# connortannahill/MM-ADMM

Hardware: AMD Instinct MI355X
Metric: ADMM iterations/sec on 1M-node 2D mesh; achieved HBM GB/s in SpMV (higher is better)
Workload: dtype f64

## Files before the change

### mm-admm_amd/csrc/host/engine.cpp

```cpp
#include <algorithm>
#include <chrono>
#include <cmath>
#include <cstring>
#include <limits>
#include <memory>
#include <mutex>
#include <string>
#include <vector>

#include "../../../include/mmx_sparse.h"
#include "../kernels/admm_kernels.h"
#include "../kernels/field_kernels.h"
#include "../kernels/quality_kernels.h"
#include "../kernels/regrid_kernels.h"
#include "../kernels/slide_kernels.h"
#include "../kernels/state_kernels.h"
#include "../kernels/transfer_kernels.h"
#include "comm.h"
#include "common.h"
#include "partition.h"
#include "slide.h"
#include "state.h"
#include "transfer.h"
#include "xup_records.h"
// ... 223 lines not shown
            std::stable_sort(ord.begin() + lo, ord.begin() + hi, [&](int a, int b) { return key[a] < key[b]; });
          }
        } else {
          std::stable_sort(ord.begin(), ord.end(), [&](int a, int b) { return key[a] < key[b]; });
        }
      };
      order(inner);
      order(bound);
      std::vector<int32_t> ord(inner);
      ord.insert(ord.end(), bound.begin(), bound.end());
      nodeOrder_.upload(ord.data(), std::max<size_t>(ord.size(), 1), st_);
      XupRecords recs;
      if (knobs_.xupRec) {
        const int ch = std::max(D == 2 ? MMX_XU_CH2D : 8, knobs_.xupCh);
        recs = build_xup_records(nl, ord.data(), plan_.incPtr.data(), plan_.incSrc.data(), invdiag.data(), ch);
        xrec_.upload(recs.rec.data(), recs.rec.size(), st_);
        xinv_.upload(recs.invdiag.data(), recs.invdiag.size(), st_);
        xslot_.upload(recs.slot.data(), recs.slot.size(), st_);
        xslotStride_ = (int)recs.stride;
        xslotCh_ = ch;
        const int chs = D == 2 ? MMX_XU_CH2D : knobs_.xupCh;
        xupTail_ = 0;
        for (int v = 0; v < nl; ++v) xupTail_ += std::max(0, plan_.incPtr[v + 1] - plan_.incPtr[v] - chs);
      }
      streamWait();
    }
    invdiag_.upload(invdiag.data(), invdiag.size(), st_);
    if (compMesh_) Vc_.upload(Vcl.data(), Vcl.size(), st_);
    uploadGridCoords();
    gvals_.upload(grid_.vals.data(), grid_.vals.size(), st_);
    if (D == 3) {
      gpad_.alloc(gvals_.n / 9 * 10);
      launch_pad_rows(gvals_.p, (long long)(gvals_.n / 9), gpad_.p, st_);
    }
    updateIso();
    Vp_.upload(Vl.data(), Vl.size(), st_);
    x_.upload(Vl.data(), Vl.size(), st_);
    xPrev_.upload(Vl.data(), Vl.size(), st_);
    xBar_.upload(Vl.data(), Vl.size(), st_);
    if (nranks_ > 1) {
      expOff_.upload(plan_.sendOff.data(), std::max<size_t>(plan_.sendOff.size(), 1), st_);
      export_.alloc((size_t)std::max<size_t>(plan_.sendOff.size(), 1) * D);
      remote_.alloc((size_t)std::max(plan_.recvRows, 1) * D);
    }
    z_.alloc((size_t)nF_ * K * (kZUInterleaved ? 2 : 1));
    gcache_.alloc((size_t)nF_ * K);
// ... 71 lines not shown
      m_.zx = zsrc;
    else
      launch_gather_z<D>(m_, zsrc, z_.p, st_);
    gcacheValid_ = false;
    if (!zFromX) m_.zx = nullptr;
    StepScalars sc{prm_.tau, prm_.dt * prm_.dt, w_, dtOverTau};
    int nbx = 0, nbp = 0;
    if (fusePred) {
      m_.predPrev = xPrev_.p;
      m_.predBar = xBar_.p;
    }
    PackZX pz;
    if (zFromX) {
      pz.F = F_.p;
      pz.zx = zsrc;
      if (fusePred) {
        pz.x = x_.p;
        pz.xPrev = xPrev_.p;
      }
    }
    xupdateHalo(sc, &nbx, false, false, pz);
    m_.predPrev = m_.predBar = nullptr;
    const bool early = tol >= 0;
    int done = 0;
    double primal = 0, dual = 0;
    const bool deferRed = !early && nIters <= kDeferMax;
    const size_t slice = maxBlocks_ * kNumPartials;
    if (deferRed && partA_.n < slice * nIters) partA_.alloc(slice * std::max(nIters, 10));
    int firstDeferred = 0;
    hipEvent_t prevEnd = nullptr;
    for (int i = 0; i < nIters; ++i) {
      hipEvent_t a0 = nullptr, a1 = nullptr, b1 = nullptr;
      if (timing) {
        a0 = prevEnd;
        if (!a0) {
          a0 = nextEvent();
          MMX_HIP(hipEventRecord(a0, st_));
        }
      }
      const bool firstProx = !hessComputed_;
      const bool swapB = prox_double_buffered(D, knobs_.prox2dWave) && hessComputed_;
      if (hessComputed_) {
        tiePar_ ^= 1;
        std::swap(m_.tieCount, m_.tieStale);
      }
      m_.gcSkip = (D == 2 && knobs_.gcSkip && !early && i == nIters - 1) ? 1 : 0;
      launch_prox<D>(m_, knobs_, !hessComputed_, gcacheValid_, early ? tol / 100 : 1e-3 / 100, x_.p, z_.p, uPtr(), B_.p,
                     swapB ? B2_.p : B_.p, partA_.p + (deferRed ? slice * i : 0), &nbp, st_);
      m_.zx = nullptr;
      if (swapB) std::swap(B_.p, B2_.p);
      gcacheValid_ = !m_.gcSkip;
      if (timing) {
        a1 = nextEvent();
        MMX_HIP(hipEventRecord(a1, st_));
      }
      hessComputed_ = true;
      stepTaken_ = true;
      const bool resid = early || i == nIters - 1;
      xupdateHalo(sc, &nbx, resid, true, PackZX{});
      if (timing) {
        b1 = nextEvent();
        MMX_HIP(hipEventRecord(b1, st_));
        timed_.push_back({a0, a1, b1});
      }
      prevEnd = b1;
      if (deferRed) {
        if (firstProx && i < nIters - 1) {
          prevEnd = nullptr;
          launch_reduce_partials(partA_.p + slice * i, nbp, res_ + (size_t)i * 2 * kNumPartials, st_, red_);
          firstDeferred = i + 1;
        } else if (i == nIters - 1) {
          const int i0 = firstProx ? i : firstDeferred;
          launch_reduce_steps(partA_.p + slice * i0, slice, nbp, partB_.p, nbx, nIters - i0,
                              res_ + (size_t)i0 * 2 * kNumPartials, st_, red_);
        }
      } else if (resid) {
        prevEnd = nullptr;
        launch_reduce_partials2(partA_.p, nbp, res_ + (size_t)i * 2 * kNumPartials, partB_.p, nbx,
                                res_ + (size_t)i * 2 * kNumPartials + kNumPartials, st_, red_);
      } else {
        prevEnd = nullptr;
        launch_reduce_partials(partA_.p, nbp, res_ + (size_t)i * 2 * kNumPartials, st_, red_);
      }
      done = i + 1;
      if (early) {
        std::vector<double> rv;
        fetchResults(res_ + (size_t)i * 2 * kNumPartials, 1, rv);
        const double* r = rv.data();
        primal = sqrt(r[kNumPartials + 2]);
        dual = sqrt(r[1]);
        if (r[4] > 0 || (primal < tol && dual < tol)) break;
      }
    }
    if (slideOn_ && !slS_.sliding.empty()) {
      launch_slide_project<D>(slX0_.p, slFaces_.p, slStarPtr_.p, slStarFace_.p, slMask_.p, slIds_.p,
                              (int)slS_.sliding.size(), x_.p, slAnchor_.p, slStepCnt_.p, st_);
      slStepValid_ = true;
    }
    MMX_HIP(hipMemcpyAsync(Vp_.p, x_.p, (size_t)nP_ * D * sizeof(double), hipMemcpyDeviceToDevice, st_));
    vpVersion_++;
    if (timing) {
      eStep1 = nextEvent();
      MMX_HIP(hipEventRecord(eStep1, st_));
    }
    fetchResults(res_, done, hostRes_);
    MMX_HIP(hipGetLastError());
    bool bad = false;
    long long bf = 0;
    int mx = 0;
    for (int i = 0; i < done; ++i) {
      const double* r = &hostRes_[(size_t)i * 2 * kNumPartials];
      bad |= r[4] > 0;
      bf += (long long)r[3];
      mx = std::max(mx, (int)r[5]);
    }
#ifdef MMX_HINT_PROBE
    {
      double hits = 0;
      for (int i = 0; i < done; ++i) hits += hostRes_[(size_t)i * 2 * kNumPartials + 2];
      fprintf(stderr, "[hint-probe] step %lld: %.0f hits of %.0f lookups in %d proxes\n", (long long)stepsTaken_, hits,
              3.0 * nF_ * done, done);
    }
// ... 215 lines not shown
    if (n) *n = nP_;
    if (ids) std::memcpy(ids, plan_.localNodes.data(), plan_.localNodes.size() * sizeof(int32_t));
  }

  void sizes(int* nP, int* nF, int* gridRows) override {
    if (nP) *nP = nP_;
    if (nF) *nF = nF_;
    if (gridRows) *gridRows = (int)(grid_.vals.size() / (D * D));
  }

  void setTiming(bool on) override {
    resolveTimed();
    timing_ = on;
  }

  void stats(mmadmm_stats* s) override {
    resolveTimed();
    *s = st_stats_;
    const double nF = nF_, nP = nP_;
    const double ts = knobs_.tslot ? 1.0 : 0.0;
    s->prox_bytes = nF * (4.0 * (D + 1) + 1 + 8.0 * (2 * K + K * K) * 2 + 8.0 * K * 2 + ts * 8.0 * K) +
                    nP * 8.0 * D;
    const double ch = D == 2 ? MMX_XU_CH2D : knobs_.xupCh;
    const double fixed = knobs_.xupRec ? nP * (4.0 * kXupRecInts + 8.0 + 4.0 * ch) + 4.0 * (double)xupTail_
                                 : 4.0 * (nP + 1) + 4.0 * (D + 1) * nF + 8.0 * nP;
    s->xupdate_bytes = fixed + (16.0 - 8.0 * ts) * K * nF + 8.0 * D * nP * 2;
    s->monitor_iso = iso_ ? 1 : 0;
    s->halo_send_bytes = 8.0 * D * (double)plan_.sendOff.size();
    s->halo_recv_bytes = nranks_ > 1 ? 8.0 * D * (double)plan_.recvRows : 0.0;
    s->interior_nodes = nInner_;
    s->overlap = knobs_.overlap;
  }

  std::string options() const override { return knobs_.text(); }

  void resetStats() override {
    resolveTimed();
    const mmadmm_stats z{};
    st_stats_ = z;
  }

  void resolveTimed() {
    if (stepEv_.empty() && timed_.empty() && exEv_.empty()) return;
    streamWait();
    float ms = 0;
    for (auto& p : stepEv_) {
      MMX_HIP(hipEventElapsedTime(&ms, p.first, p.second));
      st_stats_.t_step_ms += ms;
// ... 1382 lines not shown
    m.inc_off = incOff_.p;
    m.remote = nranks_ > 1 ? remote_.p : nullptr;
    m.tslot = knobs_.tslot ? tslot_.p : nullptr;
    m.gcache = gcache_.p;
    m.tieList = tieList_.p;
    m.tieCount = tieCount_.p + tiePar_;
    m.tieStale = tieCount_.p + (tiePar_ ^ 1);
    m.invFlag = tieCount_.p + 2;
    m.nodeOrder = nodeOrder_.p;
    m.xupLo = 0;
    m.xupHi = nP_;
    m.prox2dWave = knobs_.prox2dWave;
    m.xupSweep = knobs_.xupSweep;
    m.xupCh = knobs_.xupCh;
    m.xupEarly = knobs_.xupEarly;
    m.forceTie = knobs_.forceTie;
    m.monHint = knobs_.monHint;
    if (knobs_.xupRec) {
      m.xrec = xrec_.p;
      m.xinv = xinv_.p;
      m.xslot = xslot_.p;
      m.xslotStride = xslotStride_;
      m.xslotCh = xslotCh_;
    }
    m.invdiag = invdiag_.p;
    m.Vc = compMesh_ ? Vc_.p : nullptr;
    m.gx = gx_.p;
    m.gy = gy_.p;
    m.gz = (D == 3) ? gz_.p : gy_.p;
    m.gvals = gvals_.p;
    m.gpad = (D == 3) ? gpad_.p : nullptr;
    for (int a = 0; a < 3; ++a) m.gcell[a] = (D == 3) ? gcell_[a].p : nullptr;
    m.giso = iso_ ? giso_.p : nullptr;
    m.gnx = grid_.nx;
    m.gny = grid_.ny;
    m.gnz = grid_.nz;
    m.ghx = grid_.gx[1] - grid_.gx[0];
    m.ghy = grid_.gy[1] - grid_.gy[0];
    m.ghz = (D == 3) ? grid_.gz[1] - grid_.gz[0] : 1.0;
    m.grhx = 1.0 / m.ghx;
    m.grhy = 1.0 / m.ghy;
    m.grhz = 1.0 / m.ghz;
    const int ns[3] = {grid_.nx, grid_.ny, grid_.nz};
    double* A[3] = {&m.gax, &m.gay, &m.gaz};
    double* SP[3] = {&m.gspx, &m.gspy, &m.gspz};
    double* NS[3] = {&m.gnsx, &m.gnsy, &m.gnsz};
// ... 116 lines not shown
  DevBuf<unsigned char> rgScan_;
  size_t rgScanBytes_ = 0;
  double* rgHost_ = nullptr;
  hipStream_t st_ = nullptr;
  hipStream_t st2_ = nullptr;
  hipEvent_t evProx_ = nullptr, evEx_ = nullptr;
  int nInner_ = 0;
  std::vector<std::pair<hipEvent_t, hipEvent_t>> exEv_;
  DevBuf<int32_t> F_, incPtr_, incOff_;
  DevBuf<double> tslot_;
  DevBuf<uint8_t> sbits_, interior_;
  DevBuf<double> gcell_[3];
  DevBuf<double> giso_;
  DevBuf<int> isoFlag_;
  bool iso_ = false;
  std::vector<double> gcellH_[3];
  DevBuf<double> invdiag_, Vc_, gx_, gy_, gz_, gvals_, Vp_, x_, xPrev_, xBar_, z_, u_, gs_, B_, B2_, gcache_, gpad_;
  DevBuf<double> partA_, partB_, results_, export_, remote_, resAll_, redScratch_;
  RedWork red_;
  DevBuf<int32_t> expOff_, tieList_, nodeOrder_;
  DevBuf<int32_t> xrec_, xslot_;
  DevBuf<double> xinv_;
  int xslotStride_ = 0, xslotCh_ = 0;
  long long xupTail_ = 0;
  DevBuf<unsigned> tieCount_;
  int tiePar_ = 0;
  Comm* comm_ = nullptr;
  int rank_ = 0, nranks_ = 1;
  int resultsCap_ = 0;
  std::vector<double> hostRes_;
  DeviceMesh<D> m_{};
  bool hessComputed_ = false, stepTaken_ = false, gcacheValid_ = false;
  mmx_matrix jac_ = nullptr;
  mmx_param_iter jprm_{};
  bool beStepTaken_ = false, jacFactored_ = false;
  long long vpVersion_ = 0, jacVp_ = -1;
  double jacDt_ = 0.0;
  DevBuf<int32_t> jia_, jja_;
  DevBuf<double> jval_, jraw_, dv_, xn_, rhs_, dx_;
  DevBuf<unsigned> fdWork_;
  int maxColNodes_ = 65;
  int stepsTaken_ = 0;
  size_t maxBlocks_ = 1;
  static constexpr int kDeferMax = 64;
  bool timing_ = false;
  std::vector<hipEvent_t> evPool_;
// ... 450 lines not shown
```

### mm-admm_amd/csrc/host/knobs.h

```cpp
#pragma once
#include <climits>
#include <cstdio>
#include <cstdlib>
#include <cstring>
#include <stdexcept>
#include <string>

namespace mmx {

constexpr int kTslot2dMax = 2 * 2048 * 64;
constexpr int kXupEarlyDefault = 1;
constexpr int kRedSplitMin = 4096;
constexpr int kProxBlock = 64;
constexpr int kSweepGrid = 128;
constexpr int kFacWaveChunk = 0;
constexpr int kChainImportLat = 8;
constexpr int kFacImpRows = 384;
constexpr int kFacRMax = 4;

inline int env_int(const char* name, int dflt, int lo = INT_MIN, int hi = INT_MAX) {
  const char* e = std::getenv(name);
  if (!e) return dflt;
  const int v = std::atoi(e);
  return v < lo ? lo : v > hi ? hi : v;
// ... 50 lines not shown
    buf[n] = 0;
  }
  return (int)s.size() + 1;
}
}

#define MMX_ENGINE_KNOBS(X) \
   \
   \
  X(int, tslot, "MMX_TSLOT", nullptr, env_flag("MMX_TSLOT", D == 3 || nF <= kTslot2dMax)) \
   \
  X(int, spin, "MMX_SPIN", nullptr, env_flag("MMX_SPIN", true)) \
   \
  X(int, zx, "MMX_ZX", nullptr, env_flag("MMX_ZX", true)) \
   \
  X(int, overlap, "MMX_OVERLAP", nullptr, nranks > 1 && env_flag("MMX_OVERLAP", true)) \
   \
  X(int, fusePred, "MMX_FUSE_PRED", nullptr, env_flag("MMX_FUSE_PRED", true)) \
   \
  X(int, gcSkip, "MMX_GC_SKIP", nullptr, env_flag("MMX_GC_SKIP", true)) \
   \
  X(int, xupOrder, "MMX_XUP_ORDER", nullptr, env_int("MMX_XUP_ORDER", D == 3) == 1) \
   \
  X(int, xupRec, "MMX_XUP_REC", nullptr, env_flag("MMX_XUP_REC", true)) \
   \
  X(int, xupCh, "MMX_XUP_CH", nullptr, knobs_detail::snap_xup_ch(env_int("MMX_XUP_CH", 8))) \
   \
   \
   \
  X(int, xupSweep, "MMX_XUP_SWEEP", nullptr, env_int("MMX_XUP_SWEEP", D == 3 ? 1 : (k.xupRec ? 2 : 0), 0)) \
   \
  X(int, xupEarly, "MMX_XUP_EARLY", nullptr, env_flag("MMX_XUP_EARLY", kXupEarlyDefault != 0)) \
   \
  X(int, xupSweepResid, "MMX_XUP_SWEEP_RESID", nullptr, env_flag("MMX_XUP_SWEEP_RESID", true)) \
   \
   \
  X(int, xcdMap, "MMX_XCD_MAP", nullptr, env_int("MMX_XCD_MAP", 1)) \
   \
  X(int, prox2dWave, "MMX_PROX2D", "lds|wave", D == 2 && env_word("MMX_PROX2D", "lds|wave")) \
   \
  X(int, prox3dQuad, "MMX_PROX3D", "wave|quad", env_word("MMX_PROX3D", "wave|quad")) \
   \
  X(int, proxBlock, "MMX_PROX_BLOCK", nullptr, knobs_detail::one_of3(env_int("MMX_PROX_BLOCK", 0), 64, 128, 256, kProxBlock)) \
   \
  X(int, gradCache, "MMX_GRAD_CACHE", nullptr, env_int("MMX_GRAD_CACHE", 1)) \
   \
  X(int, forceTie, "MMX_FORCE_TIE", nullptr, env_int("MMX_FORCE_TIE", 0)) \
// ... 121 lines not shown
```

### mm-admm_amd/csrc/host/xup_records.h

```cpp
#pragma once
#include <algorithm>
#include <cstddef>
#include <cstdint>
#include <vector>

#include "../kernels/layout.h"

namespace mmx {

struct XupRecords {
  int ch = 0;
  size_t stride = 0;
  std::vector<int32_t> rec;
  std::vector<double> invdiag;
  std::vector<int32_t> slot;
};

inline XupRecords build_xup_records(int nP, const int32_t* order, const int32_t* incPtr, const int32_t* incOff,
                                    const double* invdiag, int ch) {
  XupRecords r;
  r.ch = ch;
  r.stride = (std::max<size_t>((size_t)std::max(nP, 0), 1) + kXupStridePad - 1) / kXupStridePad * kXupStridePad;
  r.rec.assign(r.stride * kXupRecInts, 0);
  r.invdiag.assign(r.stride, 0.0);
  r.slot.assign((size_t)ch * r.stride, 0);
  for (int p = 0; p < nP; ++p) {
    const int32_t v = order ? order[p] : p;
    const int32_t b = incPtr[v], e = incPtr[v + 1];
    r.rec[(size_t)p * kXupRecInts + 0] = v;
    r.rec[(size_t)p * kXupRecInts + 1] = b;
    r.rec[(size_t)p * kXupRecInts + 2] = e;
    r.invdiag[p] = invdiag[v];
    if (e > b)
      for (int j = 0; j < ch; ++j) r.slot[(size_t)j * r.stride + p] = incOff[std::min(b + j, e - 1)];
  }
  return r;
}

}
```

### mm-admm_amd/csrc/kernels/admm_kernels.h

```cpp
#pragma once
#include <hip/hip_runtime.h>
#include <stdint.h>

#include "../host/knobs.h"
#include "layout.h"

namespace mmx {

constexpr int kNumPartials = kLayoutPartials;

template <int D>
struct DeviceMesh {
  int nP, nF;
  const int* F;
  const uint8_t* sbits;
  const uint8_t* nodeInterior;
  const int* inc_ptr;
  const int* inc_off;
  const double* remote;
  double* tslot;
  const double* zx;
  double* predPrev;
  double* predBar;
  double* gcache;
// ... 9 lines not shown
  int xupLo, xupHi;
  const double* invdiag;
  const int* xrec;
  const double* xinv;
  const int* xslot;
  int xslotStride, xslotCh;
  int xupEarly;
  int gcSkip;
  const double* Vc;
  const double* gx;
  const double* gy;
  const double* gz;
  const double* gvals;
  const double* gpad;
  const double* gcell[3];
  const double* giso;
  int gnx, gny, gnz;
  double ghx, ghy, ghz, grhx, grhy, grhz;
  double gax, gay, gaz, gspx, gspy, gspz, gnsx, gnsy, gnsz, grnsx, grnsy, grnsz;
  double Ehat[9];
  double powd, w;
  int compMesh;
  int prox2dWave;
};

struct StepScalars {
  double tau, dtsq, w, dt_over_tau;
};

template <int D>
void launch_gather_z(const DeviceMesh<D>& m, const double* x, double* z, hipStream_t st);
template <int D>
void launch_grad_simplex(const DeviceMesh<D>& m, const double* x, double* gs, bool zeroFixed,
                         double* partials, int* nblocks, hipStream_t st);
template <int D>
void launch_predict(const DeviceMesh<D>& m, const EngineKnobs& k, int mode, const double* gs, double* x, double* xPrev,
                    double* xBar, double dt_over_tau, hipStream_t st);
template <int D>
void launch_xupdate(const DeviceMesh<D>& m, const EngineKnobs& k, const StepScalars& sc, const double* xBar,
                    const double* z, const double* u, double* x, double* partials, int* nblocks,
                    bool resid, hipStream_t st, bool useTslot = false);
void launch_pad_rows(const double* vals, long long rows, double* pad, hipStream_t st);
template <int D>
void launch_iso_compact(const double* vals, long long points, double* iso, int* notIso, hipStream_t st);
template <int D>
void launch_bkinv_identity(int nF, double* B, hipStream_t st);
// ... 51 lines not shown
```

### mm-admm_amd/csrc/kernels/admm_kernels_step.hip

```cpp
#include "admm_common.h"

namespace mmx {
template <int D>
__global__ void __launch_bounds__(kBlock) k_gather_z(DeviceMesh<D> m, const double* __restrict__ x,
                                                      double* __restrict__ z) {
  constexpr int K = D * (D + 1);
  const int s = blockIdx.x * kBlock + threadIdx.x;
  if (s >= m.nF) return;
  int f[D + 1];
  loadVerts<D>(m, s, f);
  double v[K];
  gatherX<D>(x, f, v);
#pragma unroll
  for (int i = 0; i < K; ++i) z[zu_base<D>(s) + zu_i<D>(i)] = v[i];
}

template <int D, int ISO = -1>
__global__ void __launch_bounds__(kBlock) k_grad_simplex(DeviceMesh<D> m, const double* __restrict__ x,
                                                          double* __restrict__ gs, int zeroFixedRows,
                                                          double* __restrict__ partials) {
  constexpr int K = D * (D + 1);
  const int s = blockIdx.x * kBlock + threadIdx.x;
  double pv[5] = {0, 0, 0, 0, 0};
  if (s < m.nF) {
// ... 30 lines not shown
    for (int t = b; t < e; ++t) {
      const int off = m.inc_off[t];
      const double* src = (off >= 0) ? gs + off : m.remote + (size_t)(-1 - off) * D;
#pragma unroll
      for (int c = 0; c < D; ++c) g[c] += src[c];
    }
#pragma unroll
    for (int c = 0; c < D; ++c) xb[c] = xv[c] - dt_over_tau * g[c];
  } else {
#pragma unroll
    for (int c = 0; c < D; ++c) xb[c] = 2 * xv[c] - xPrev[(size_t)v * D + c];
  }
#pragma unroll
  for (int c = 0; c < D; ++c) {
    xBar[(size_t)v * D + c] = xb[c];
    xPrev[(size_t)v * D + c] = xv[c];
  }
}

template <int CH>
struct XupHead {
  int v, b, e;
  double inv;
  int off[CH];
};
template <int D, int CH>
__device__ __forceinline__ void xup_head_rec(const DeviceMesh<D>& m, int idx, XupHead<CH>& h) {
  const int* r = m.xrec + (size_t)idx * kXupRecInts;
  h.v = r[0];
  h.b = r[1];
  h.e = r[2];
  h.inv = m.xinv[idx];
#pragma unroll
  for (int j = 0; j < CH; ++j) h.off[j] = m.xslot[(size_t)j * m.xslotStride + idx];
}
template <int D, int CH>
__device__ __forceinline__ void xup_head_csr(const DeviceMesh<D>& m, int idx, XupHead<CH>& h) {
  h.v = m.nodeOrder ? m.nodeOrder[idx] : idx;
  h.b = m.inc_ptr[h.v];
  h.e = m.inc_ptr[h.v + 1];
  h.inv = m.invdiag[h.v];
#pragma unroll
  for (int j = 0; j < CH; ++j) h.off[j] = (h.e > h.b) ? m.inc_off[min(h.b + j, h.e - 1)] : 0;
}
template <int D, bool RESID, bool TS, int CH = 8, bool ZX = false, bool PRED = false, bool REM = false>
__device__ __forceinline__ void xupdate_node(const DeviceMesh<D>& m, const StepScalars& sc,
                                             const double* __restrict__ xBar, const double* __restrict__ z,
                                             const double* __restrict__ u, double* __restrict__ x,
                                             const XupHead<CH>& h, double (&pv)[3]) {
  {
    const int v = h.v, b = h.b, e = h.e;
    double acc[D];
#pragma unroll
    for (int c = 0; c < D; ++c) acc[c] = 0.0;
    double xb[D], zn[D];
    if constexpr (PRED) {
      double xv[D];
#pragma unroll
      for (int c = 0; c < D; ++c) {
        xv[c] = x[(size_t)v * D + c];
        xb[c] = 2 * xv[c] - m.predPrev[(size_t)v * D + c];
      }
#pragma unroll
      for (int c = 0; c < D; ++c) {
        m.predBar[(size_t)v * D + c] = xb[c];
        m.predPrev[(size_t)v * D + c] = xv[c];
      }
    } else {
#pragma unroll
      for (int c = 0; c < D; ++c) xb[c] = xBar[(size_t)v * D + c];
    }
    constexpr bool zv0 = ZX && !TS;
    if constexpr (zv0) {
      if constexpr (PRED) {
#pragma unroll
        for (int c = 0; c < D; ++c) zn[c] = xb[c];
      } else {
#pragma unroll
        for (int c = 0; c < D; ++c) zn[c] = m.zx[(size_t)v * D + c];
      }
    }
    const double inv = h.inv;
    auto addChunk = [&](int t0, const int(&off)[CH]) {
      double zv[CH][D], uv[CH][D];
#pragma unroll
      for (int j = 0; j < CH; ++j) {
        const bool loc = off[j] >= 0;
        if constexpr (TS) {
          const double* pt = loc ? m.tslot + off[j] : m.remote + (size_t)(-1 - off[j]) * D;
#pragma unroll
          for (int c = 0; c < D; ++c) zv[j][c] = pt[c];
        } else {
          const double* pz = loc ? z + zu_off<D>(off[j]) : m.remote + (size_t)(-1 - off[j]) * D;
          const double* pu = loc ? u + zu_off<D>(off[j]) : pz;
#pragma unroll
          for (int c = 0; c < D; ++c) {
            if constexpr (zv0 && REM)
              zv[j][c] = loc ? zn[c] : pz[c];
            else if constexpr (zv0)
              zv[j][c] = zn[c];
            else
              zv[j][c] = pz[c];
            uv[j][c] = pu[c];
          }
        }
      }
#pragma unroll
      for (int j = 0; j < CH; ++j) {
        if (t0 + j < e) {
#pragma unroll
          for (int c = 0; c < D; ++c) {
            if constexpr (TS)
              acc[c] += zv[j][c];
            else
              acc[c] += (off[j] >= 0) ? sc.w * (sc.w * (zv[j][c] - uv[j][c])) : zv[j][c];
          }
        }
      }
    };
    if (b < e) addChunk(b, h.off);
    for (int t0 = b + CH; t0 < e; t0 += CH) {
      int off[CH];
#pragma unroll
      for (int j = 0; j < CH; ++j) off[j] = m.inc_off[min(t0 + j, e - 1)];
      addChunk(t0, off);
    }
    double xn[D];
#pragma unroll
    for (int c = 0; c < D; ++c) {
      xn[c] = ((sc.tau * xb[c]) + sc.dtsq * acc[c]) * inv;
      x[(size_t)v * D + c] = xn[c];
    }
    if constexpr (RESID) {
      double r2 = 0.0;
      auto residChunk = [&](int t0, const int(&off)[CH]) {
        double zv[CH][D];
#pragma unroll
        for (int j = 0; j < CH; ++j) {
          const double* pz = z + zu_off<D>(off[j] >= 0 ? off[j] : 0);
#pragma unroll
          for (int c = 0; c < D; ++c) zv[j][c] = pz[c];
        }
#pragma unroll
        for (int j = 0; j < CH; ++j) {
          if (t0 + j < e && off[j] >= 0) {
#pragma unroll
            for (int c = 0; c < D; ++c) {
              const double d = xn[c] - zv[j][c];
              r2 += d * d;
            }
          }
        }
      };
      if (b < e) residChunk(b, h.off);
      for (int t0 = b + CH; t0 < e; t0 += CH) {
        int off[CH];
#pragma unroll
        for (int j = 0; j < CH; ++j) off[j] = m.inc_off[min(t0 + j, e - 1)];
        residChunk(t0, off);
      }
      pv[2] = r2;
    }
  }
}
template <int D, int CH, bool REC>
__device__ __forceinline__ void xup_head(const DeviceMesh<D>& m, int idx, XupHead<CH>& h) {
  if constexpr (REC)
    xup_head_rec<D, CH>(m, idx, h);
  else
    xup_head_csr<D, CH>(m, idx, h);
}
template <int D, bool RESID, bool TS, bool ZX = false, bool PRED = false, bool REM = false, bool REC = false>
__global__ void __launch_bounds__(kBlock) k_xupdate(DeviceMesh<D> m, StepScalars sc,
                                                     const double* __restrict__ xBar,
                                                     const double* __restrict__ z,
                                                     const double* __restrict__ u, double* __restrict__ x,
                                                     double* __restrict__ partials, int xcd) {
  constexpr int CH = (D == 2 ? MMX_XU_CH2D : 8);
  const int lb = logical_block(xcd);
  const int idx = m.xupLo + lb * kBlock + threadIdx.x;
  double pv[3] = {0, 0, 0};
  if (idx < m.xupHi) {
    XupHead<CH> h;
    xup_head<D, CH, REC>(m, idx, h);
    xupdate_node<D, RESID, TS, CH, ZX, PRED, REM>(m, sc, xBar, z, u, x, h, pv);
  }
  if constexpr (RESID) block_partials<3>(pv, partials, lb);
}
template <int D, bool TS, int CH, bool RESID = false, bool REC = false, bool EARLY = false>
__global__ void __launch_bounds__(kBlock) k_xupdate_sweep(DeviceMesh<D> m, StepScalars sc,
                                                           const double* __restrict__ xBar,
                                                           const double* __restrict__ z, const double* __restrict__ u,
                                                           double* __restrict__ x, int n8, double* __restrict__ partials) {
  static_assert(REC || !EARLY, "the early request reads the records");
  const int c = (int)(blockIdx.x % 8), w = (int)(blockIdx.x / 8), per = (int)(gridDim.x / 8);
  const int lo = m.xupLo + c * n8, hi = min(lo + n8, m.xupHi);
  double pv[3], r2 = 0.0;
  int idx = lo + w * kBlock + (int)threadIdx.x;
  if constexpr (EARLY) {
    XupHead<CH> cur, nxt;
    if (idx < hi) xup_head<D, CH, true>(m, idx, cur);
    nxt = cur;
    for (; idx < hi; idx += per * kBlock) {
      if (idx + per * kBlock < hi) xup_head<D, CH, true>(m, idx + per * kBlock, nxt);
      __builtin_amdgcn_sched_barrier(0);
      xupdate_node<D, RESID, TS, CH>(m, sc, xBar, z, u, x, cur, pv);
      if constexpr (RESID) r2 += pv[2];
      cur = nxt;
    }
  } else {
    for (; idx < hi; idx += per * kBlock) {
      XupHead<CH> h;
      xup_head<D, CH, REC>(m, idx, h);
      xupdate_node<D, RESID, TS, CH>(m, sc, xBar, z, u, x, h, pv);
      if constexpr (RESID) r2 += pv[2];
    }
  }
  if constexpr (RESID) {
    double q[3] = {0.0, 0.0, r2};
    block_partials<3>(q, partials, (int)blockIdx.x);
  }
}

template <int D, int ISO = -1>
__global__ void __launch_bounds__(kBlock) k_energy(DeviceMesh<D> m, const double* __restrict__ x,
                                                    double* __restrict__ partials) {
  constexpr int K = D * (D + 1);
  const int s = blockIdx.x * kBlock + threadIdx.x;
  double pv[5] = {0, 0, 0, 0, 0};
  if (s < m.nF) {
    int f[D + 1];
    loadVerts<D>(m, s, f);
    double z[K], xi[K], Igt;
    gatherX<D>(x, f, z);
    loadXi<D>(m, f, xi);
    const double e = blockGrad<D, false, false>(gridOf<D, ISO>(m), constsOf<D>(m), z, xi, nullptr, nullptr, Igt);
    pv[0] = e;
// ... 165 lines not shown
                       zeroFixedRows ? 1 : 0, partials);
  });
}
template <int D>
void launch_predict(const DeviceMesh<D>& m, const EngineKnobs& k, int mode, const double* gs, double* x,
                    double* xPrev, double* xBar, double dt_over_tau, hipStream_t st) {
  if (m.nP == 0) return;
  hipLaunchKernelGGL(k_predict<D>, dim3(nblk_xcd(m.nP, k.xcdMap)), dim3(kBlock), 0, st, m, mode, gs, x, xPrev, xBar,
                     dt_over_tau, k.xcdMap);
}
template <int D>
void launch_xupdate(const DeviceMesh<D>& m, const EngineKnobs& k, const StepScalars& sc, const double* xBar,
                    const double* z, const double* u, double* x, double* partials, int* nblocks, bool resid,
                    hipStream_t st, bool useTslot) {
  const int nsub = m.xupHi - m.xupLo;
  *nblocks = nblk_xcd(nsub, k.xcdMap);
  if (nsub <= 0) {
    *nblocks = 0;
    return;
  }
  const bool ts = useTslot && m.tslot;
  const bool rem = m.remote != nullptr;
  const bool rec = m.xrec != nullptr;
  auto needCols = [&](int ch) {
    if (rec && m.xslotCh < ch) throw std::logic_error("launch_xupdate: the slot table has fewer columns than the chunk");
  };
  if (m.zx && !resid && !ts) {
    needCols(D == 2 ? MMX_XU_CH2D : 8);
    dispatch_bool(m.predBar != nullptr, [&](auto pred) {
      dispatch_bool(rem, [&](auto r) {
        dispatch_bool(rec, [&](auto rc) {
          hipLaunchKernelGGL(
              (k_xupdate<D, false, false, true, decltype(pred)::value, decltype(r)::value, decltype(rc)::value>),
              dim3(*nblocks), dim3(kBlock), 0, st, m, sc, xBar, z, u, x, partials, k.xcdMap);
        });
      });
    });
    return;
  }
  if (m.predBar || m.predPrev)
    throw std::logic_error("launch_xupdate: predBar set for an x-update that cannot fuse predictX");
  const bool sweepResid = resid && ts && k.xupSweepResid;
  if (m.xupSweep > 0 && (!resid || sweepResid)) {
    const int n8 = ((nsub + kBlock - 1) / kBlock + 7) / 8 * kBlock;
    const dim3 g(256 * m.xupSweep);
    auto sweep = [&](auto tsT, auto chT, auto residT, double* part) {
      constexpr bool TS = decltype(tsT)::value, RS = decltype(residT)::value;
      constexpr int CH = decltype(chT)::value;
      needCols(CH);
      if (rec && m.xupEarly)
        hipLaunchKernelGGL((k_xupdate_sweep<D, TS, CH, RS, true, true>), g, dim3(kBlock), 0, st, m, sc, xBar, z, u, x, n8,
                           part);
      else if (rec)
        hipLaunchKernelGGL((k_xupdate_sweep<D, TS, CH, RS, true, false>), g, dim3(kBlock), 0, st, m, sc, xBar, z, u, x, n8,
                           part);
      else
        hipLaunchKernelGGL((k_xupdate_sweep<D, TS, CH, RS>), g, dim3(kBlock), 0, st, m, sc, xBar, z, u, x, n8, part);
    };
    using T = std::true_type;
    using F = std::false_type;
    if (sweepResid) {
      *nblocks = (int)g.x;
      sweep(T{}, std::integral_constant<int, 8>{}, T{}, partials);
    } else if (ts && m.xupCh >= 24)
      sweep(T{}, std::integral_constant<int, 24>{}, F{}, nullptr);
    else if (ts && m.xupCh >= 16)
      sweep(T{}, std::integral_constant<int, 16>{}, F{}, nullptr);
    else if (ts)
      sweep(T{}, std::integral_constant<int, 8>{}, F{}, nullptr);
    else
      sweep(F{}, std::integral_constant<int, (D == 2 ? MMX_XU_CH2D : 8)>{}, F{}, nullptr);
    return;
  }
  needCols(D == 2 ? MMX_XU_CH2D : 8);
  dispatch_bool(resid, [&](auto r) {
    dispatch_bool(ts, [&](auto t) {
      dispatch_bool(rec, [&](auto rc) {
        hipLaunchKernelGGL((k_xupdate<D, decltype(r)::value, decltype(t)::value, false, false, false, decltype(rc)::value>),
                           dim3(*nblocks), dim3(kBlock), 0, st, m, sc, xBar, z, u, x, partials, k.xcdMap);
      });
    });
  });
}
template <int D>
void launch_energy(const DeviceMesh<D>& m, const double* x, double* partials, int* nblocks, hipStream_t st) {
  *nblocks = nblk(m.nF);
  if (m.nF == 0) return;
  dispatch_iso<D>(m, [&](auto iso) {
    hipLaunchKernelGGL((k_energy<D, decltype(iso)::value>), dim3(*nblocks), dim3(kBlock), 0, st, m, x, partials);
  });
}
template <int D>
void launch_euler_apply(const DeviceMesh<D>& m, const EngineKnobs& k, const double* gs, double* x, double dt_over_tau,
                        hipStream_t st) {
  if (m.nP == 0) return;
  hipLaunchKernelGGL(k_euler_apply<D>, dim3(nblk_xcd(m.nP, k.xcdMap)), dim3(kBlock), 0, st, m, gs, x, dt_over_tau,
                     k.xcdMap);
}
static bool split_ok(const RedWork& w, int nblocks) { return w.scratch && nblocks >= w.splitMin; }
static void reduce_split(const double* partA, size_t stride, int nbA, int nA, double* outA, size_t outStride,
// ... 52 lines not shown
```

### mm-admm_amd/csrc/kernels/layout.h

```cpp
#pragma once

#ifndef MMX_ZU_INTER
#define MMX_ZU_INTER 0
#endif
#ifndef MMX_SPMV_TILE
#define MMX_SPMV_TILE 2048
#endif
#ifndef MMX_SPMV_BLOCK
#define MMX_SPMV_BLOCK 256
#endif
#ifndef MMX_B3_PAIRS
#define MMX_B3_PAIRS 1
#endif
#ifndef MMX_CHAIN_VEC
#define MMX_CHAIN_VEC 1
#endif
#ifndef MMX_CHAIN_CODE16
#define MMX_CHAIN_CODE16 1
#endif
#ifndef MMX_XU_CH2D
#define MMX_XU_CH2D 6
#endif

namespace mmx {
constexpr unsigned kXupRecInts = 3;
constexpr unsigned kXupStridePad = 64;
constexpr unsigned kLayoutPartials = 6;
constexpr unsigned kLayoutBkinvBlock = 64;
constexpr unsigned kLayoutWord = 0x4d000000u | ((unsigned)(MMX_ZU_INTER != 0) << 0) |
                                 ((unsigned)(MMX_CHAIN_VEC != 0) << 1) | ((unsigned)(MMX_CHAIN_CODE16 != 0) << 2) |
                                 (((unsigned)MMX_SPMV_TILE / 256u & 0xFu) << 4) |
                                 (((unsigned)MMX_SPMV_BLOCK / 64u & 0xFu) << 8) | ((kLayoutPartials & 0xFu) << 12) |
                                 ((kLayoutBkinvBlock / 64u & 0x3u) << 16) | ((unsigned)(MMX_B3_PAIRS != 0) << 18) |
                                 ((unsigned)(kXupRecInts == 3 && kXupStridePad == 64) << 19) |
                                 (((unsigned)MMX_XU_CH2D & 0xFu) << 20);
}
```

Baseline: 2679.

## Pack 2D x-update records into compressed 20-byte entries with class-indexed invdiag

Adds a packed per-node record format for the 2D x-update: the node id, the base offset and five 16-bit delta offsets fit in an int4 plus one word, and invdiag is replaced by a small class-table index. Nodes that do not fit fall back to the wide records. This shrinks the index bytes streamed per node. It also fuses the final Vp copy into the residual x-update and keeps z values in registers for the residual pass instead of reloading them. The cost is extra decode arithmetic, more template variants and a fallback branch per node.

```diff
diff --git a/mm-admm_amd/csrc/host/engine.cpp b/mm-admm_amd/csrc/host/engine.cpp
--- a/mm-admm_amd/csrc/host/engine.cpp
+++ b/mm-admm_amd/csrc/host/engine.cpp
@@ -269,6 +269,16 @@
         const int chs = D == 2 ? MMX_XU_CH2D : knobs_.xupCh;
         xupTail_ = 0;
         for (int v = 0; v < nl; ++v) xupTail_ += std::max(0, plan_.incPtr[v + 1] - plan_.incPtr[v] - chs);
+        xupPacked_ = D == 2 && MMX_XU_CH2D == (int)kXupPackCh &&
+                     (knobs_.xupRec == 3 || (knobs_.xupRec == 1 && nF_ > kTslot2dMax));
+        if (xupPacked_) {
+          const XupPacked pk = build_xup_packed(nl, ord.data(), plan_.incPtr.data(), plan_.incSrc.data(), invdiag.data(), D);
+          xpq_.upload(pk.q.data(), pk.q.size(), st_);
+          xpw_.upload(pk.w.data(), pk.w.size(), st_);
+          xcls_.upload(pk.cls.data(), pk.cls.size(), st_);
+          xupWide_ = (long long)pk.nWide;
+          xupPackTail_ = (long long)pk.nTail;
+        }
       }
       streamWait();
     }
@@ -386,6 +396,7 @@
     xupdateHalo(sc, &nbx, false, false, pz);
     m_.predPrev = m_.predBar = nullptr;
     const bool early = tol >= 0;
+    const bool sliding = slideOn_ && !slS_.sliding.empty();
     int done = 0;
     double primal = 0, dual = 0;
     const bool deferRed = !early && nIters <= kDeferMax;
@@ -421,7 +432,9 @@
       hessComputed_ = true;
       stepTaken_ = true;
       const bool resid = early || i == nIters - 1;
+      m_.xCopy = (resid && !sliding) ? Vp_.p : nullptr;
       xupdateHalo(sc, &nbx, resid, true, PackZX{});
+      m_.xCopy = nullptr;
       if (timing) {
         b1 = nextEvent();
         MMX_HIP(hipEventRecord(b1, st_));
@@ -456,12 +469,12 @@
         if (r[4] > 0 || (primal < tol && dual < tol)) break;
       }
     }
-    if (slideOn_ && !slS_.sliding.empty()) {
+    if (sliding) {
       launch_slide_project<D>(slX0_.p, slFaces_.p, slStarPtr_.p, slStarFace_.p, slMask_.p, slIds_.p,
                               (int)slS_.sliding.size(), x_.p, slAnchor_.p, slStepCnt_.p, st_);
       slStepValid_ = true;
     }
-    MMX_HIP(hipMemcpyAsync(Vp_.p, x_.p, (size_t)nP_ * D * sizeof(double), hipMemcpyDeviceToDevice, st_));
+    if (sliding) MMX_HIP(hipMemcpyAsync(Vp_.p, x_.p, (size_t)nP_ * D * sizeof(double), hipMemcpyDeviceToDevice, st_));
     vpVersion_++;
     if (timing) {
       eStep1 = nextEvent();
@@ -723,8 +736,12 @@
     s->prox_bytes = nF * (4.0 * (D + 1) + 1 + 8.0 * (2 * K + K * K) * 2 + 8.0 * K * 2 + ts * 8.0 * K) +
                     nP * 8.0 * D;
     const double ch = D == 2 ? MMX_XU_CH2D : knobs_.xupCh;
-    const double fixed = knobs_.xupRec ? nP * (4.0 * kXupRecInts + 8.0 + 4.0 * ch) + 4.0 * (double)xupTail_
-                                 : 4.0 * (nP + 1) + 4.0 * (D + 1) * nF + 8.0 * nP;
+    const double wide = 4.0 * kXupRecInts + 8.0 + 4.0 * ch;
+    const bool packed = xupPacked_ && !knobs_.tslot;
+    const double fixed = packed            ? nP * (double)kXupPackBytes + wide * (double)xupWide_ + 4.0 * (double)xupPackTail_ +
+                                                 4.0 * (double)xupTail_
+                         : knobs_.xupRec ? nP * wide + 4.0 * (double)xupTail_
+                                         : 4.0 * (nP + 1) + 4.0 * (D + 1) * nF + 8.0 * nP;
     s->xupdate_bytes = fixed + (16.0 - 8.0 * ts) * K * nF + 8.0 * D * nP * 2;
     s->monitor_iso = iso_ ? 1 : 0;
     s->halo_send_bytes = 8.0 * D * (double)plan_.sendOff.size();
@@ -2153,6 +2170,11 @@
       m.xslot = xslot_.p;
       m.xslotStride = xslotStride_;
       m.xslotCh = xslotCh_;
+      if (xupPacked_) {
+        m.xpq = xpq_.p;
+        m.xpw = xpw_.p;
+        m.xcls = xcls_.p;
+      }
     }
     m.invdiag = invdiag_.p;
     m.Vc = compMesh_ ? Vc_.p : nullptr;
@@ -2315,6 +2337,11 @@
   DevBuf<int32_t> xrec_, xslot_;
   DevBuf<double> xinv_;
   int xslotStride_ = 0, xslotCh_ = 0;
+  DevBuf<int32_t> xpq_;
+  DevBuf<uint32_t> xpw_;
+  DevBuf<double> xcls_;
+  bool xupPacked_ = false;
+  long long xupWide_ = 0, xupPackTail_ = 0;
   long long xupTail_ = 0;
   DevBuf<unsigned> tieCount_;
   int tiePar_ = 0;
diff --git a/mm-admm_amd/csrc/host/knobs.h b/mm-admm_amd/csrc/host/knobs.h
--- a/mm-admm_amd/csrc/host/knobs.h
+++ b/mm-admm_amd/csrc/host/knobs.h
@@ -96,7 +96,10 @@
    \
   X(int, xupOrder, "MMX_XUP_ORDER", nullptr, env_int("MMX_XUP_ORDER", D == 3) == 1) \
    \
-  X(int, xupRec, "MMX_XUP_REC", nullptr, env_flag("MMX_XUP_REC", true)) \
+   \
+   \
+   \
+  X(int, xupRec, "MMX_XUP_REC", nullptr, env_int("MMX_XUP_REC", 1, 0, 3)) \
    \
   X(int, xupCh, "MMX_XUP_CH", nullptr, knobs_detail::snap_xup_ch(env_int("MMX_XUP_CH", 8))) \
    \
diff --git a/mm-admm_amd/csrc/host/xup_records.h b/mm-admm_amd/csrc/host/xup_records.h
--- a/mm-admm_amd/csrc/host/xup_records.h
+++ b/mm-admm_amd/csrc/host/xup_records.h
@@ -2,6 +2,7 @@
 #include <algorithm>
 #include <cstddef>
 #include <cstdint>
+#include <cstring>
 #include <vector>
 
 #include "../kernels/layout.h"
@@ -37,4 +38,97 @@
   return r;
 }
 
+struct XupPacked {
+  size_t stride = 0;
+  std::vector<int32_t> q;
+  std::vector<uint32_t> w;
+  std::vector<double> cls;
+  size_t nWide = 0;
+  size_t nTail = 0;
+};
+
+inline XupPacked build_xup_packed(int nP, const int32_t* order, const int32_t* incPtr, const int32_t* incOff,
+                                  const double* invdiag, int dim) {
+  const int ch = (int)kXupPackCh;
+  XupPacked r;
+  r.stride = (std::max<size_t>((size_t)std::max(nP, 0), 1) + kXupStridePad - 1) / kXupStridePad * kXupStridePad;
+  r.q.assign(r.stride * 4, 0);
+  r.w.assign(r.stride, 0);
+  auto bits = [](double d) {
+    uint64_t u;
+    static_assert(sizeof u == sizeof d, "double is 64 bits");
+    std::memcpy(&u, &d, sizeof u);
+    return u;
+  };
+  std::vector<uint64_t> seen;
+  std::vector<uint8_t> cls((size_t)std::max(nP, 0), 0);
+  bool clsOk = true;
+  for (int p = 0; p < nP && clsOk; ++p) {
+    const uint64_t u = bits(invdiag[order ? order[p] : p]);
+    size_t c = 0;
+    while (c < seen.size() && seen[c] != u) ++c;
+    if (c == seen.size()) {
+      if (seen.size() == kXupPackMaxCls) {
+        clsOk = false;
+        break;
+      }
+      seen.push_back(u);
+    }
+    cls[p] = (uint8_t)c;
+  }
+  if (!clsOk) seen.clear();
+  r.cls.assign(std::max<size_t>(seen.size(), 1), 0.0);
+  for (size_t c = 0; c < seen.size(); ++c) std::memcpy(&r.cls[c], &seen[c], sizeof(double));
+  for (int p = 0; p < nP; ++p) {
+    const int32_t v = order ? order[p] : p;
+    const int32_t b = incPtr[v], e = incPtr[v + 1];
+    bool fits = clsOk && e - b <= (int32_t)kXupPackMaxCount;
+    for (int32_t t = b; t < e && fits; ++t) fits = incOff[t] >= 0;
+    int32_t off[kXupPackCh] = {0, 0, 0, 0, 0, 0};
+    int32_t d[kXupPackCh] = {0, 0, 0, 0, 0, 0};
+    if (fits && e > b) {
+      for (int j = 0; j < ch; ++j) off[j] = incOff[std::min(b + j, e - 1)];
+      for (int j = 1; j < ch && fits; ++j) {
+        const int64_t delta = (int64_t)off[j] - off[0];
+        fits = delta % dim == 0 && delta / dim >= -32768 && delta / dim <= 32767;
+        d[j] = (int32_t)(delta / dim);
+      }
+    }
+    if (!fits) {
+      r.w[p] = kXupPackWide;
+      r.nWide++;
+      continue;
+    }
+    auto lo16 = [](int32_t x) { return (uint32_t)x & 0xFFFFu; };
+    r.q[(size_t)p * 4 + 0] = v;
+    r.q[(size_t)p * 4 + 1] = off[0];
+    r.q[(size_t)p * 4 + 2] = (int32_t)(lo16(d[1]) | lo16(d[2]) << 16);
+    r.q[(size_t)p * 4 + 3] = (int32_t)(lo16(d[3]) | lo16(d[4]) << 16);
+    r.w[p] = lo16(d[5]) | (uint32_t)(e - b) << 16 | (uint32_t)cls[p] << 24;
+    if (e - b > ch) r.nTail++;
+  }
+  return r;
 }
+
+struct XupDecoded {
+  int32_t v = 0, count = 0, cls = 0;
+  int32_t off[kXupPackCh] = {0, 0, 0, 0, 0, 0};
+};
+inline bool decode_xup_packed(const XupPacked& r, size_t p, int dim, XupDecoded& o) {
+  const int32_t* q = &r.q[p * 4];
+  const uint32_t w = r.w[p];
+  if (w & kXupPackWide) return false;
+  auto s16 = [](uint32_t x) { return (int32_t)(int16_t)(uint16_t)(x & 0xFFFFu); };
+  o.v = q[0];
+  o.count = (int32_t)(w >> 16 & kXupPackMaxCount);
+  o.cls = (int32_t)(w >> 24);
+  o.off[0] = q[1];
+  o.off[1] = q[1] + dim * s16((uint32_t)q[2]);
+  o.off[2] = q[1] + dim * s16((uint32_t)q[2] >> 16);
+  o.off[3] = q[1] + dim * s16((uint32_t)q[3]);
+  o.off[4] = q[1] + dim * s16((uint32_t)q[3] >> 16);
+  o.off[5] = q[1] + dim * s16(w);
+  return true;
+}
+
+}
diff --git a/mm-admm_amd/csrc/kernels/admm_kernels.h b/mm-admm_amd/csrc/kernels/admm_kernels.h
--- a/mm-admm_amd/csrc/kernels/admm_kernels.h
+++ b/mm-admm_amd/csrc/kernels/admm_kernels.h
@@ -55,6 +55,10 @@
   double powd, w;
   int compMesh;
   int prox2dWave;
+  const int* xpq;
+  const unsigned* xpw;
+  const double* xcls;
+  double* xCopy;
 };
 
 struct StepScalars {
diff --git a/mm-admm_amd/csrc/kernels/admm_kernels_step.hip b/mm-admm_amd/csrc/kernels/admm_kernels_step.hip
--- a/mm-admm_amd/csrc/kernels/admm_kernels_step.hip
+++ b/mm-admm_amd/csrc/kernels/admm_kernels_step.hip
@@ -1,4 +1,8 @@
 #include "admm_common.h"
+
+#ifndef MMX_XUP_KEEPZ
+#define MMX_XUP_KEEPZ 1
+#endif
 
 namespace mmx {
 template <int D>
@@ -76,8 +80,18 @@
 struct XupHead {
   int v, b, e;
   double inv;
+  int key;
   int off[CH];
 };
+struct XupRaw {
+  int4 q;
+  unsigned w;
+};
+template <int D>
+__device__ __forceinline__ void xup_raw_load(const DeviceMesh<D>& m, int idx, XupRaw& r) {
+  r.q = reinterpret_cast<const int4*>(m.xpq)[idx];
+  r.w = m.xpw[idx];
+}
 template <int D, int CH>
 __device__ __forceinline__ void xup_head_rec(const DeviceMesh<D>& m, int idx, XupHead<CH>& h) {
   const int* r = m.xrec + (size_t)idx * kXupRecInts;
@@ -89,6 +103,25 @@
   for (int j = 0; j < CH; ++j) h.off[j] = m.xslot[(size_t)j * m.xslotStride + idx];
 }
 template <int D, int CH>
+__device__ __forceinline__ void xup_head_packed(const DeviceMesh<D>& m, int idx, const XupRaw& r, XupHead<CH>& h) {
+  static_assert(CH == (int)kXupPackCh, "the packed records hold the first kXupPackCh slots");
+  if (r.w & kXupPackWide) {
+    xup_head_rec<D, CH>(m, idx, h);
+    h.key = -1 - idx;
+    return;
+  }
+  h.v = r.q.x;
+  h.b = 0;
+  h.e = (int)(r.w >> 16 & kXupPackMaxCount);
+  h.key = (int)(r.w >> 24);
+  h.off[0] = r.q.y;
+  h.off[1] = r.q.y + D * (int)(short)(r.q.z & 0xFFFF);
+  h.off[2] = r.q.y + D * (r.q.z >> 16);
+  h.off[3] = r.q.y + D * (int)(short)(r.q.w & 0xFFFF);
+  h.off[4] = r.q.y + D * (r.q.w >> 16);
+  h.off[5] = r.q.y + D * (int)(short)(r.w & 0xFFFFu);
+}
+template <int D, int CH>
 __device__ __forceinline__ void xup_head_csr(const DeviceMesh<D>& m, int idx, XupHead<CH>& h) {
   h.v = m.nodeOrder ? m.nodeOrder[idx] : idx;
   h.b = m.inc_ptr[h.v];
@@ -97,7 +130,7 @@
 #pragma unroll
   for (int j = 0; j < CH; ++j) h.off[j] = (h.e > h.b) ? m.inc_off[min(h.b + j, h.e - 1)] : 0;
 }
-template <int D, bool RESID, bool TS, int CH = 8, bool ZX = false, bool PRED = false, bool REM = false>
+template <int D, bool RESID, bool TS, int CH = 8, bool ZX = false, bool PRED = false, bool REM = false, bool PK = false>
 __device__ __forceinline__ void xupdate_node(const DeviceMesh<D>& m, const StepScalars& sc,
                                              const double* __restrict__ xBar, const double* __restrict__ z,
                                              const double* __restrict__ u, double* __restrict__ x,
@@ -134,8 +167,14 @@
         for (int c = 0; c < D; ++c) zn[c] = m.zx[(size_t)v * D + c];
       }
     }
-    const double inv = h.inv;
-    auto addChunk = [&](int t0, const int(&off)[CH]) {
+    double inv = h.inv;
+    if constexpr (PK) inv = *(h.key >= 0 ? m.xcls + h.key : m.xinv + (-1 - h.key));
+    int tb = b;
+    if constexpr (PK)
+      if (e - b > CH) tb = m.inc_ptr[v];
+    constexpr bool keepZ = RESID && !TS && MMX_XUP_KEEPZ;
+    double zkeep[keepZ ? CH : 1][D];
+    auto addChunk = [&](int t0, const int(&off)[CH], bool first) {
       double zv[CH][D], uv[CH][D];
 #pragma unroll
       for (int j = 0; j < CH; ++j) {
@@ -171,19 +210,31 @@
           }
         }
       }
+      if constexpr (keepZ)
+        if (first) {
+#pragma unroll
+          for (int j = 0; j < CH; ++j)
+#pragma unroll
+            for (int c = 0; c < D; ++c) zkeep[j][c] = zv[j][c];
+        }
     };
-    if (b < e) addChunk(b, h.off);
+    if (b < e) addChunk(b, h.off, true);
+    const int* tailOff = m.inc_off + (tb - b);
     for (int t0 = b + CH; t0 < e; t0 += CH) {
       int off[CH];
 #pragma unroll
-      for (int j = 0; j < CH; ++j) off[j] = m.inc_off[min(t0 + j, e - 1)];
-      addChunk(t0, off);
+      for (int j = 0; j < CH; ++j) off[j] = tailOff[min(t0 + j, e - 1)];
+      addChunk(t0, off, false);
     }
     double xn[D];
 #pragma unroll
     for (int c = 0; c < D; ++c) {
       xn[c] = ((sc.tau * xb[c]) + sc.dtsq * acc[c]) * inv;
       x[(size_t)v * D + c] = xn[c];
+    }
+    if (m.xCopy) {
+#pragma unroll
+      for (int c = 0; c < D; ++c) m.xCopy[(size_t)v * D + c] = xn[c];
     }
     if constexpr (RESID) {
       double r2 = 0.0;
@@ -206,25 +257,44 @@
           }
         }
       };
-      if (b < e) residChunk(b, h.off);
+      if constexpr (keepZ) {
+        if (b < e) {
+#pragma unroll
+          for (int j = 0; j < CH; ++j) {
+            if (b + j < e && h.off[j] >= 0) {
+#pragma unroll
+              for (int c = 0; c < D; ++c) {
+                const double d = xn[c] - zkeep[j][c];
+                r2 += d * d;
+              }
+            }
+          }
+        }
+      } else {
+        if (b < e) residChunk(b, h.off);
+      }
       for (int t0 = b + CH; t0 < e; t0 += CH) {
         int off[CH];
 #pragma unroll
-        for (int j = 0; j < CH; ++j) off[j] = m.inc_off[min(t0 + j, e - 1)];
+        for (int j = 0; j < CH; ++j) off[j] = tailOff[min(t0 + j, e - 1)];
         residChunk(t0, off);
       }
       pv[2] = r2;
     }
   }
 }
-template <int D, int CH, bool REC>
+template <int D, int CH, int REC>
 __device__ __forceinline__ void xup_head(const DeviceMesh<D>& m, int idx, XupHead<CH>& h) {
-  if constexpr (REC)
+  if constexpr (REC == 2) {
+    XupRaw r;
+    xup_raw_load<D>(m, idx, r);
+    xup_head_packed<D, CH>(m, idx, r, h);
+  } else if constexpr (REC == 1)
     xup_head_rec<D, CH>(m, idx, h);
   else
     xup_head_csr<D, CH>(m, idx, h);
 }
-template <int D, bool RESID, bool TS, bool ZX = false, bool PRED = false, bool REM = false, bool REC = false>
+template <int D, bool RESID, bool TS, bool ZX = false, bool PRED = false, bool REM = false, int REC = 0>
 __global__ void __launch_bounds__(kBlock) k_xupdate(DeviceMesh<D> m, StepScalars sc,
                                                      const double* __restrict__ xBar,
                                                      const double* __restrict__ z,
@@ -237,26 +307,39 @@
   if (idx < m.xupHi) {
     XupHead<CH> h;
     xup_head<D, CH, REC>(m, idx, h);
-    xupdate_node<D, RESID, TS, CH, ZX, PRED, REM>(m, sc, xBar, z, u, x, h, pv);
+    xupdate_node<D, RESID, TS, CH, ZX, PRED, REM, REC == 2>(m, sc, xBar, z, u, x, h, pv);
   }
   if constexpr (RESID) block_partials<3>(pv, partials, lb);
 }
-template <int D, bool TS, int CH, bool RESID = false, bool REC = false, bool EARLY = false>
+template <int D, bool TS, int CH, bool RESID = false, int REC = 0, bool EARLY = false>
 __global__ void __launch_bounds__(kBlock) k_xupdate_sweep(DeviceMesh<D> m, StepScalars sc,
                                                            const double* __restrict__ xBar,
                                                            const double* __restrict__ z, const double* __restrict__ u,
                                                            double* __restrict__ x, int n8, double* __restrict__ partials) {
-  static_assert(REC || !EARLY, "the early request reads the records");
+  static_assert(REC != 0 || !EARLY, "the early request reads the records");
   const int c = (int)(blockIdx.x % 8), w = (int)(blockIdx.x / 8), per = (int)(gridDim.x / 8);
   const int lo = m.xupLo + c * n8, hi = min(lo + n8, m.xupHi);
   double pv[3], r2 = 0.0;
   int idx = lo + w * kBlock + (int)threadIdx.x;
-  if constexpr (EARLY) {
-    XupHead<CH> cur, nxt;
-    if (idx < hi) xup_head<D, CH, true>(m, idx, cur);
+  if constexpr (EARLY && REC == 2) {
+    XupRaw cur, nxt;
+    if (idx < hi) xup_raw_load<D>(m, idx, cur);
     nxt = cur;
     for (; idx < hi; idx += per * kBlock) {
-      if (idx + per * kBlock < hi) xup_head<D, CH, true>(m, idx + per * kBlock, nxt);
+      if (idx + per * kBlock < hi) xup_raw_load<D>(m, idx + per * kBlock, nxt);
+      __builtin_amdgcn_sched_barrier(0);
+      XupHead<CH> h;
+      xup_head_packed<D, CH>(m, idx, cur, h);
+      xupdate_node<D, RESID, TS, CH, false, false, false, true>(m, sc, xBar, z, u, x, h, pv);
+      if constexpr (RESID) r2 += pv[2];
+      cur = nxt;
+    }
+  } else if constexpr (EARLY) {
+    XupHead<CH> cur, nxt;
+    if (idx < hi) xup_head<D, CH, 1>(m, idx, cur);
+    nxt = cur;
+    for (; idx < hi; idx += per * kBlock) {
+      if (idx + per * kBlock < hi) xup_head<D, CH, 1>(m, idx + per * kBlock, nxt);
       __builtin_amdgcn_sched_barrier(0);
       xupdate_node<D, RESID, TS, CH>(m, sc, xBar, z, u, x, cur, pv);
       if constexpr (RESID) r2 += pv[2];
@@ -266,7 +349,7 @@
     for (; idx < hi; idx += per * kBlock) {
       XupHead<CH> h;
       xup_head<D, CH, REC>(m, idx, h);
-      xupdate_node<D, RESID, TS, CH>(m, sc, xBar, z, u, x, h, pv);
+      xupdate_node<D, RESID, TS, CH, false, false, false, REC == 2>(m, sc, xBar, z, u, x, h, pv);
       if constexpr (RESID) r2 += pv[2];
     }
   }
@@ -478,6 +561,15 @@
   const bool ts = useTslot && m.tslot;
   const bool rem = m.remote != nullptr;
   const bool rec = m.xrec != nullptr;
+  auto dispatch_rec = [&](auto chT, auto&& f) {
+    constexpr int CH = decltype(chT)::value;
+    if constexpr (D == 2 && CH == (int)kXupPackCh) {
+      if (rec && m.xpq) return f(std::integral_constant<int, 2>{});
+    }
+    if (rec) return f(std::integral_constant<int, 1>{});
+    return f(std::integral_constant<int, 0>{});
+  };
+  using ChNode = std::integral_constant<int, (D == 2 ? MMX_XU_CH2D : 8)>;
   auto needCols = [&](int ch) {
     if (rec && m.xslotCh < ch) throw std::logic_error("launch_xupdate: the slot table has fewer columns than the chunk");
   };
@@ -485,7 +577,7 @@
     needCols(D == 2 ? MMX_XU_CH2D : 8);
     dispatch_bool(m.predBar != nullptr, [&](auto pred) {
       dispatch_bool(rem, [&](auto r) {
-        dispatch_bool(rec, [&](auto rc) {
+        dispatch_rec(ChNode{}, [&](auto rc) {
           hipLaunchKernelGGL(
               (k_xupdate<D, false, false, true, decltype(pred)::value, decltype(r)::value, decltype(rc)::value>),
               dim3(*nblocks), dim3(kBlock), 0, st, m, sc, xBar, z, u, x, partials, k.xcdMap);
@@ -504,14 +596,18 @@
       constexpr bool TS = decltype(tsT)::value, RS = decltype(residT)::value;
       constexpr int CH = decltype(chT)::value;
       needCols(CH);
-      if (rec && m.xupEarly)
-        hipLaunchKernelGGL((k_xupdate_sweep<D, TS, CH, RS, true, true>), g, dim3(kBlock), 0, st, m, sc, xBar, z, u, x, n8,
+      dispatch_rec(chT, [&](auto rc) {
+        constexpr int RC = decltype(rc)::value;
+        if constexpr (RC != 0) {
+          if (m.xupEarly) {
+            hipLaunchKernelGGL((k_xupdate_sweep<D, TS, CH, RS, RC, true>), g, dim3(kBlock), 0, st, m, sc, xBar, z, u, x,
+                               n8, part);
+            return;
+          }
+        }
+        hipLaunchKernelGGL((k_xupdate_sweep<D, TS, CH, RS, RC, false>), g, dim3(kBlock), 0, st, m, sc, xBar, z, u, x, n8,
                            part);
-      else if (rec)
-        hipLaunchKernelGGL((k_xupdate_sweep<D, TS, CH, RS, true, false>), g, dim3(kBlock), 0, st, m, sc, xBar, z, u, x, n8,
-                           part);
-      else
-        hipLaunchKernelGGL((k_xupdate_sweep<D, TS, CH, RS>), g, dim3(kBlock), 0, st, m, sc, xBar, z, u, x, n8, part);
+      });
     };
     using T = std::true_type;
     using F = std::false_type;
@@ -531,7 +627,7 @@
   needCols(D == 2 ? MMX_XU_CH2D : 8);
   dispatch_bool(resid, [&](auto r) {
     dispatch_bool(ts, [&](auto t) {
-      dispatch_bool(rec, [&](auto rc) {
+      dispatch_rec(ChNode{}, [&](auto rc) {
         hipLaunchKernelGGL((k_xupdate<D, decltype(r)::value, decltype(t)::value, false, false, false, decltype(rc)::value>),
                            dim3(*nblocks), dim3(kBlock), 0, st, m, sc, xBar, z, u, x, partials, k.xcdMap);
       });
diff --git a/mm-admm_amd/csrc/kernels/layout.h b/mm-admm_amd/csrc/kernels/layout.h
--- a/mm-admm_amd/csrc/kernels/layout.h
+++ b/mm-admm_amd/csrc/kernels/layout.h
@@ -25,6 +25,11 @@
 namespace mmx {
 constexpr unsigned kXupRecInts = 3;
 constexpr unsigned kXupStridePad = 64;
+constexpr unsigned kXupPackCh = 6;
+constexpr unsigned kXupPackBytes = 20;
+constexpr unsigned kXupPackWide = 1u << 23;
+constexpr unsigned kXupPackMaxCount = 127;
+constexpr unsigned kXupPackMaxCls = 255;
 constexpr unsigned kLayoutPartials = 6;
 constexpr unsigned kLayoutBkinvBlock = 64;
 constexpr unsigned kLayoutWord = 0x4d000000u | ((unsigned)(MMX_ZU_INTER != 0) << 0) |
@@ -32,6 +37,6 @@
                                  (((unsigned)MMX_SPMV_TILE / 256u & 0xFu) << 4) |
                                  (((unsigned)MMX_SPMV_BLOCK / 64u & 0xFu) << 8) | ((kLayoutPartials & 0xFu) << 12) |
                                  ((kLayoutBkinvBlock / 64u & 0x3u) << 16) | ((unsigned)(MMX_B3_PAIRS != 0) << 18) |
-                                 ((unsigned)(kXupRecInts == 3 && kXupStridePad == 64) << 19) |
+                                 ((unsigned)(kXupRecInts == 3 && kXupStridePad == 64 && kXupPackBytes == 20) << 19) |
                                  (((unsigned)MMX_XU_CH2D & 0xFu) << 20);
 }
```

Measured after the change: 2637. 0.984x the previous value.
